# ViktorNfa/bluerov2_dynamics

Measured on AMD Instinct MI355X. Metric: rk4_rollout_steps_per_s, higher is better.
Workload: dtype f64; 1 GPU; BASELINE config 2: 65536 trajectories/GPU x 5000 RK4 steps, thruster model, dt=0.02, iid U(-1,1) commands (splitmix64 stream 0x5EED), layout tpb, all states stored; trajectories_per_gpu=65536, horizon=5000, parallelism=1 x independent shards, no collective

## Files before the change

bluerov2_dynamics_amd/csrc/brov2_fast.h:

```cpp
#pragma once
#include "brov2_device.h"

namespace brov {

struct FastParams {
    double E[12];
    double da[6], db[6];
    double G[5];
    double lc[4][3];
    double ld[4];
    double Tm[6][8];
    double minv[6];
    double poly[5];
    double A1[9], b1[3];
    double A4[9], b4[3];
    double Ob[9];
    double al4[3];
    double Aw4[9], bw4[3];
    double g1[3];
    double XY[4];
    double cur[3];
    int has_current;
    int has_xy;
    int tm_dense;
    int obs_bad;
};

typedef const FastParams __attribute__((address_space(4)))* CFP;
__device__ __forceinline__ CFP as_constant(const FastParams* g) { return (CFP)(unsigned long long)g; }

template <bool RES>
struct HotConstsT {
    static constexpr bool RESIDENT = RES;
    double E[12], db[6];
    double da[6], G[5], ld[4], al4[3];
    double tk[2];
};
typedef HotConstsT<false> HotConsts;
typedef HotConstsT<true> HotConstsResident;

#ifndef BROV_CLAMP_BRANCH
#define BROV_CLAMP_BRANCH 1
#endif
#ifndef BROV_PSI_FRAME
#define BROV_PSI_FRAME 1
#endif
#define BROV_PIN_V(x) asm volatile("" : "+v"(x))
#define BROV_PIN_S(x) asm volatile("" : "+s"(x))
#define BROV_FORM_HERE(r) asm volatile("" : "+v"(r))
#define BROV_SC(h, p, f) (HC::RESIDENT ? (h).f : (p)->f)

template <bool RES>
__device__ __forceinline__ void load_hot(CFP pp, HotConstsT<RES>& h) {
    const auto& p = *pp;
#pragma unroll
    for (int i = 0; i < 12; ++i) { h.E[i] = p.E[i]; BROV_PIN_V(h.E[i]); }
#pragma unroll
    for (int i = 0; i < 6; ++i) { h.db[i] = p.db[i]; BROV_PIN_V(h.db[i]); }
    if constexpr (RES) {
#pragma unroll
        for (int i = 0; i < 6; ++i) { h.da[i] = p.da[i]; BROV_PIN_S(h.da[i]); }
#pragma unroll
        for (int i = 0; i < 5; ++i) { h.G[i] = p.G[i]; BROV_PIN_S(h.G[i]); }
#pragma unroll
        for (int i = 0; i < 4; ++i) { h.ld[i] = p.ld[i]; BROV_PIN_S(h.ld[i]); }
#pragma unroll
        for (int i = 0; i < 3; ++i) { h.al4[i] = p.al4[i]; BROV_PIN_S(h.al4[i]); }
        h.tk[0] = -1.98412698298579493134e-04; BROV_PIN_V(h.tk[0]);
        h.tk[1] = 2.48015872894767294178e-05;  BROV_PIN_V(h.tk[1]);
    }
}

template <bool GENERIC, class HC>
__device__ __forceinline__ const double* trig_consts(const HC& h) {
    if constexpr (HC::RESIDENT && !GENERIC) return h.tk; else return nullptr;
}

__device__ __forceinline__ CFP relaunder(CFP p) {
    asm volatile("" : "+s"(p));
    return p;
}

__device__ __forceinline__ void sincos_fast(double x, double& s, double& c, const double2* __restrict__ qt, const double* kv = nullptr) {
    const double S7 = kv ? kv[0] : -1.98412698298579493134e-04, C8 = kv ? kv[1] : 2.48015872894767294178e-05;
    const double kf = rint(x * 6.36619772367581382433e-01);
    double r = fma(-kf, 1.57079632673412561417e+00, x);
    r = fma(-kf, 6.07710050630396597660e-11, r);
    r = fma(-kf, 2.02226624879595063154e-21, r);
    const int q = (int)kf;
    const double z = r * r;
    double ps = fma(z, 1.58969099521155010221e-10, -2.50507602534068634195e-08);
    ps = fma(z, ps, 2.75573137070700676789e-06);
    ps = fma(z, ps, S7);
    ps = fma(z, ps, 8.33333333332248946124e-03);
    ps = fma(z, ps, -1.66666666666666324348e-01);
    const double sr = fma(z * r, ps, r);
    double pc = fma(z, -1.13596475577881948265e-11, 2.08757232129817482790e-09);
    pc = fma(z, pc, -2.75573143513906633035e-07);
    pc = fma(z, pc, C8);
    pc = fma(z, pc, -1.38888888888741095749e-03);
    pc = fma(z, pc, 4.16666666666666019037e-02);
    const double cr = fma(z * z, pc, fma(-0.5, z, 1.0));
    const double2 t = qt[q & 3];
    s = fma(cr, t.y, sr * t.x);
    c = fma(-sr, t.y, cr * t.x);
}

__device__ __forceinline__ void init_quadrant_table(double2* qt) {
    if (threadIdx.x < 4) {
        const int q = threadIdx.x;
        qt[q] = make_double2(q == 0 ? 1.0 : (q == 2 ? -1.0 : 0.0), q == 1 ? 1.0 : (q == 3 ? -1.0 : 0.0));
    }
}

struct Trig { double sphi, cphi, sth, cth, spsi, cpsi; };

__device__ __forceinline__ void trig_full(const double* ang, Trig& t, const double2* __restrict__ qt, const double* kv = nullptr) {
    sincos_fast(ang[0], t.sphi, t.cphi, qt, kv);
    sincos_fast(ang[1], t.sth, t.cth, qt, kv);
    sincos_fast(ang[2], t.spsi, t.cpsi, qt, kv);
}

template <bool SHORT = false, bool LEAN = false>
__device__ __forceinline__ void trig_delta(const Trig& b, double d[3], Trig& t, double* dpsi = nullptr, const double* kv = nullptr) {
    constexpr int K0 = SHORT ? 4 : 3;
    const double S7 = kv ? kv[0] : -1.98412698298579493134e-04, C8 = kv ? kv[1] : 2.48015872894767294178e-05;
    double dcopy[3] = {d[0], d[1], d[2]};
    double* dd = LEAN ? d : dcopy;
    int k = 0;
    const double m = fmax(fmax(fabs(d[0]), fabs(d[1])), fabs(d[2]));
    const bool far = !(m <= (SHORT ? 0.0625 : 0.125));
    if (far) {
        double mf = m;
        if constexpr (LEAN) asm volatile("; trig_delta range extension, rare" : "+v"(mf));
        int e;
        (void)frexp(mf, &e);
        k = e + K0;
        double sc = ldexp(1.0, -k);
        if (!(mf < 0x1p37)) { sc = __builtin_nan(""); k = 0; }
#pragma unroll
        for (int i = 0; i < 3; ++i) dd[i] *= sc;
    }
    double sd[3], cm[3];
#pragma unroll
    for (int i = 0; i < 3; ++i) {
        const double z = dd[i] * dd[i];
        double ps, pc;
        if constexpr (SHORT) {
            ps = fma(z, S7, 8.33333333332248946124e-03);
            pc = fma(z, C8, -1.38888888888741095749e-03);
        } else {
            ps = fma(z, 2.75573137070700676789e-06, S7);
            ps = fma(z, ps, 8.33333333332248946124e-03);
            pc = fma(z, -2.75573143513906633035e-07, C8);
            pc = fma(z, pc, -1.38888888888741095749e-03);
        }
        ps = fma(z, ps, -1.66666666666666324348e-01);
        sd[i] = fma(z * dd[i], ps, dd[i]);
        pc = fma(z, pc, 4.16666666666666019037e-02);
        pc = fma(z, pc, -0.5);
        cm[i] = z * pc;
    }
    auto doubling = [&](int n) {
        for (int j = 0; j < n; ++j) {
#pragma unroll
            for (int i = 0; i < 3; ++i) {
                const double t2 = sd[i] + sd[i];
                const double s2 = fma(t2, cm[i], t2);
                cm[i] = -(t2 * sd[i]);
                sd[i] = s2;
            }
        }
    };
    if constexpr (LEAN) {
        if (far) {
            double mf = m;
            asm volatile("; trig_delta doubling, rare" : "+v"(mf));
            int e;
            (void)frexp(mf, &e);
            doubling((mf < 0x1p37) ? e + K0 : 0);
        }
    } else doubling(k);
    t.sphi = fma(b.cphi, sd[0], fma(b.sphi, cm[0], b.sphi)); t.cphi = fma(-b.sphi, sd[0], fma(b.cphi, cm[0], b.cphi));
    t.sth = fma(b.cth, sd[1], fma(b.sth, cm[1], b.sth));     t.cth = fma(-b.sth, sd[1], fma(b.cth, cm[1], b.cth));
    t.spsi = fma(b.cpsi, sd[2], fma(b.spsi, cm[2], b.spsi)); t.cpsi = fma(-b.spsi, sd[2], fma(b.cpsi, cm[2], b.cpsi));
    if (dpsi) { dpsi[0] = sd[2]; dpsi[1] = cm[2]; }
}

#ifndef BROV_TRIG_SHORT
#define BROV_TRIG_SHORT 1
#endif
__device__ __forceinline__ double recip_fast(double x) {
    double y = __builtin_amdgcn_rcp(x);
    double e = fma(-x, y, 1.0);
    y = fma(y, e, y);
    e = fma(-x, y, 1.0);
    return fma(y, e, y);
}

template <bool GENERIC, class HC>
__device__ __forceinline__ void nu_dot_fast(const HC& h, CFP p, const double R[9], const double nu[6],
                                            const double a[6], double sth, double ctsp, double ctcp, double out[6]) {
    const double u = nu[0], v = nu[1], w = nu[2], pp = nu[3], q = nu[4], r = nu[5];
    double nr0 = u, nr1 = v, nr2 = w;
    if (GENERIC && p->has_current) {
        nr0 -= fma(R[6], p->cur[2], fma(R[3], p->cur[1], R[0] * p->cur[0]));
        nr1 -= fma(R[7], p->cur[2], fma(R[4], p->cur[1], R[1] * p->cur[0]));
        nr2 -= fma(R[8], p->cur[2], fma(R[5], p->cur[1], R[2] * p->cur[0]));
    }
    double o0 = fma(-h.E[0], w * q, a[0]);  o0 = fma(h.E[1], v * r, o0);
    double o1 = fma(-h.E[2], u * r, a[1]);  o1 = fma(h.E[3], w * pp, o1);
    double o2 = fma(-h.E[4], v * pp, a[2]); o2 = fma(h.E[5], u * q, o2);
    double o3 = fma(-h.E[6], v * w, a[3]);  o3 = fma(-h.E[7], q * r, o3);
    double o4 = fma(-h.E[8], u * w, a[4]);  o4 = fma(-h.E[9], pp * r, o4);
    double o5 = fma(-h.E[10], u * v, a[5]); o5 = fma(-h.E[11], pp * q, o5);
    o0 = fma(-fma(h.db[0], fabs(nr0), BROV_SC(h, p, da[0])), nr0, o0);
    o1 = fma(-fma(h.db[1], fabs(nr1), BROV_SC(h, p, da[1])), nr1, o1);
    o2 = fma(-fma(h.db[2], fabs(nr2), BROV_SC(h, p, da[2])), nr2, o2);
    o3 = fma(-fma(h.db[3], fabs(pp), BROV_SC(h, p, da[3])), pp, o3);
    o4 = fma(-fma(h.db[4], fabs(q), BROV_SC(h, p, da[4])), q, o4);
    o5 = fma(-fma(h.db[5], fabs(r), BROV_SC(h, p, da[5])), r, o5);
    o0 = fma(-BROV_SC(h, p, G[0]), sth, o0);
    o1 = fma(BROV_SC(h, p, G[1]), ctsp, o1);
    o2 = fma(BROV_SC(h, p, G[2]), ctcp, o2);
    o3 = fma(BROV_SC(h, p, G[3]), ctsp, o3);
    o4 = fma(BROV_SC(h, p, G[4]), sth, o4);
    if (GENERIC && p->has_xy) {
        o3 = fma(-p->XY[0], ctcp, o3);
        o4 = fma(p->XY[1], ctcp, o4);
        o5 = fma(-p->XY[2], ctsp, o5);
        o5 = fma(-p->XY[3], sth, o5);
    }
    out[0] = o0; out[1] = o1; out[2] = o2; out[3] = o3; out[4] = o4; out[5] = o5;
}

template <bool GENERIC, class HC, bool PFRAME = false>
__device__ __forceinline__ void rhs_fast_euler(const HC& h, CFP p, const double x[12], const double a[6], double xd[12], const Trig& tg) {
    const double sphi = tg.sphi, cphi = tg.cphi, sth = tg.sth, cth = tg.cth, spsi = tg.spsi, cpsi = tg.cpsi;
    const double* nu = x + 6;
    const double ctsp = cth * sphi, ctcp = cth * cphi;
    if constexpr (GENERIC) {
        double R[9];
        const double ss = sth * sphi, sc = sth * cphi;
        R[0] = cpsi * cth; R[1] = fma(cpsi, ss, -(spsi * cphi)); R[2] = fma(cpsi, sc, spsi * sphi);
        R[3] = spsi * cth; R[4] = fma(spsi, ss, cpsi * cphi);    R[5] = fma(spsi, sc, -(cpsi * sphi));
        R[6] = -sth;       R[7] = ctsp;                          R[8] = ctcp;
        nu_dot_fast<true>(h, p, R, nu, a, sth, ctsp, ctcp, xd + 6);
#pragma unroll
        for (int i = 0; i < 3; ++i) xd[i] = fma(R[3 * i + 2], nu[2], fma(R[3 * i + 1], nu[1], R[3 * i] * nu[0]));
    } else {
        nu_dot_fast<false>(h, p, nullptr, nu, a, sth, ctsp, ctcp, xd + 6);
        const double y1 = fma(cphi, nu[1], -(sphi * nu[2])), z1 = fma(sphi, nu[1], cphi * nu[2]);
        const double x2 = fma(cth, nu[0], sth * z1), z2 = fma(cth, z1, -(sth * nu[0]));
        if constexpr (PFRAME) { xd[0] = x2; xd[1] = y1; }
        else {
            xd[0] = fma(cpsi, x2, -(spsi * y1));
            xd[1] = fma(spsi, x2, cpsi * y1);
        }
        xd[2] = z2;
    }
#if BROV_CLAMP_BRANCH
    double ic = recip_fast(cth);
    if (__builtin_amdgcn_ballot_w64(fabs(cth) < 1e-7) != 0) {
        asm volatile("; cos(theta) clamp, rare" ::: "memory");
        if (fabs(cth) < 1e-7) ic = recip_fast(1e-7 * ((cth > 0.0) - (cth < 0.0)));
    }
#else
    double cc = cth;
    if (fabs(cc) < 1e-7) cc = 1e-7 * ((cc > 0.0) - (cc < 0.0));
    const double ic = recip_fast(cc);
#endif
    const double m = fma(sphi, nu[4], cphi * nu[5]);
    xd[3] = fma(sth * ic, m, nu[3]);
    xd[4] = fma(cphi, nu[4], -(sphi * nu[5]));
    xd[5] = ic * m;
}

template <bool GENERIC, class HC>
__device__ __forceinline__ void rhs_fast_quat(const HC& h, CFP p, const double x[13], const double a[6], double xd[13]) {
    double q[4] = {x[3], x[4], x[5], x[6]};
    quat_normalize(q);
    const double qw = q[0], qx = q[1], qy = q[2], qz = q[3];
    double R[9];
    R[0] = 1.0 - 2.0 * fma(qy, qy, qz * qz); R[1] = 2.0 * fma(qx, qy, -(qz * qw));    R[2] = 2.0 * fma(qx, qz, qy * qw);
    R[3] = 2.0 * fma(qx, qy, qz * qw);       R[4] = 1.0 - 2.0 * fma(qx, qx, qz * qz); R[5] = 2.0 * fma(qy, qz, -(qx * qw));
    R[6] = 2.0 * fma(qx, qz, -(qy * qw));    R[7] = 2.0 * fma(qy, qz, qx * qw);       R[8] = 1.0 - 2.0 * fma(qx, qx, qy * qy);
    const double* nu = x + 7;
    nu_dot_fast<GENERIC>(h, p, R, nu, a, -R[6], R[7], R[8], xd + 7);
#pragma unroll
    for (int i = 0; i < 3; ++i) xd[i] = fma(R[3 * i + 2], nu[2], fma(R[3 * i + 1], nu[1], R[3 * i] * nu[0]));
    const double wx = nu[3], wy = nu[4], wz = nu[5];
    xd[3] = 0.5 * (-(qx * wx) - qy * wy - qz * wz);
    xd[4] = 0.5 * (qw * wx + qy * wz - qz * wy);
    xd[5] = 0.5 * (qw * wy - qx * wz + qz * wx);
    xd[6] = 0.5 * (qw * wz + qx * wy - qy * wx);
}

__device__ __forceinline__ void rhs_di_euler(const double x[12], const double a[6], double xd[12], const Trig& tg) {
    const double sphi = tg.sphi, cphi = tg.cphi, sth = tg.sth, cth = tg.cth, spsi = tg.spsi, cpsi = tg.cpsi;
    const double* v = x + 6;
    const double y1 = fma(cphi, v[1], -(sphi * v[2])), z1 = fma(sphi, v[1], cphi * v[2]);
    const double x2 = fma(cth, v[0], sth * z1);
    xd[0] = fma(cpsi, x2, -(spsi * y1));
    xd[1] = fma(spsi, x2, cpsi * y1);
    xd[2] = fma(cth, z1, -(sth * v[0]));
#pragma unroll
    for (int i = 0; i < 3; ++i) xd[3 + i] = x[9 + i];
#pragma unroll
    for (int i = 0; i < 6; ++i) xd[6 + i] = a[i];
}
__device__ __forceinline__ void rhs_di_quat(const double x[13], const double a[6], double xd[13]) {
    double q[4] = {x[3], x[4], x[5], x[6]};
    quat_normalize(q);
    const double qw = q[0], qx = q[1], qy = q[2], qz = q[3];
    const double R0 = 1.0 - 2.0 * fma(qy, qy, qz * qz), R1 = 2.0 * fma(qx, qy, -(qz * qw)), R2 = 2.0 * fma(qx, qz, qy * qw);
    const double R3 = 2.0 * fma(qx, qy, qz * qw), R4 = 1.0 - 2.0 * fma(qx, qx, qz * qz), R5 = 2.0 * fma(qy, qz, -(qx * qw));
    const double R6 = 2.0 * fma(qx, qz, -(qy * qw)), R7 = 2.0 * fma(qy, qz, qx * qw), R8 = 1.0 - 2.0 * fma(qx, qx, qy * qy);
    const double* v = x + 7;
    xd[0] = fma(R2, v[2], fma(R1, v[1], R0 * v[0]));
    xd[1] = fma(R5, v[2], fma(R4, v[1], R3 * v[0]));
    xd[2] = fma(R8, v[2], fma(R7, v[1], R6 * v[0]));
    const double wx = x[10], wy = x[11], wz = x[12];
    xd[3] = 0.5 * (-(qx * wx) - qy * wy - qz * wz);
    xd[4] = 0.5 * (qw * wx + qy * wz - qz * wy);
    xd[5] = 0.5 * (qw * wy - qx * wz + qz * wx);
    xd[6] = 0.5 * (qw * wz + qx * wy - qy * wx);
#pragma unroll
    for (int i = 0; i < 6; ++i) xd[7 + i] = a[i];
}

template <int MODEL, bool GENERIC, class HC, bool PFRAME = false>
__device__ __forceinline__ void rhs_fast(const HC& h, CFP p, const double* x, const double a[6], double* xd, const Trig& tg) {
    if constexpr (MODEL == MODEL_DI_WRENCH_QUAT) rhs_di_quat(x, a, xd);
    else if constexpr (model_is_di(MODEL)) rhs_di_euler(x, a, xd, tg);
    else if constexpr (MODEL == MODEL_WRENCH_QUAT) rhs_fast_quat<GENERIC>(h, p, x, a, xd);
    else rhs_fast_euler<GENERIC, HC, PFRAME>(h, p, x, a, xd, tg);
}

struct LagZ {
    double z[6][3];
    __device__ __forceinline__ void zero() {
#pragma unroll
        for (int k = 0; k < 6; ++k) { z[k][0] = 0.0; z[k][1] = 0.0; z[k][2] = 0.0; }
    }
    __device__ __forceinline__ void from_thrusters(CFP p, const double X[8][3]) {
#pragma unroll
        for (int k = 0; k < 6; ++k)
#pragma unroll
            for (int j = 0; j < 3; ++j) {
                double a = p->Tm[k][0] * X[0][j];
#pragma unroll
                for (int i = 1; i < 8; ++i) a = fma(p->Tm[k][i], X[i][j], a);
                z[k][j] = a;
            }
    }
    __device__ __forceinline__ void accel_after(CFP p, int s, const double acmd[6], double a[6]) const {
        const double c0 = p->lc[s - 1][0], c1 = p->lc[s - 1][1], c2 = p->lc[s - 1][2], d = p->ld[s - 1];
#pragma unroll
        for (int k = 0; k < 6; ++k) a[k] = fma(c2, z[k][2], fma(c1, z[k][1], fma(c0, z[k][0], d * acmd[k])));
    }
    __device__ __forceinline__ void to_observer(CFP p) {
#pragma unroll
        for (int k = 0; k < 6; ++k) {
            const double a0 = z[k][0], a1 = z[k][1], a2 = z[k][2];
            z[k][0] = fma(p->Ob[2], a2, fma(p->Ob[1], a1, p->Ob[0] * a0));
            z[k][1] = fma(p->Ob[5], a2, fma(p->Ob[4], a1, p->Ob[3] * a0));
            z[k][2] = fma(p->Ob[8], a2, fma(p->Ob[7], a1, p->Ob[6] * a0));
        }
    }
    template <class HC>
    __device__ __forceinline__ void obs_accel_after(const HC& h, CFP p, int s, const double acmd[6], double a[6]) const {
        if (s <= 3) {
            const double d = BROV_SC(h, p, ld[s - 1]);
#pragma unroll
            for (int k = 0; k < 6; ++k) a[k] = fma(d, acmd[k], z[k][s - 1]);
        } else {
            const double c0 = BROV_SC(h, p, al4[0]), c1 = BROV_SC(h, p, al4[1]), c2 = BROV_SC(h, p, al4[2]), d = BROV_SC(h, p, ld[3]);
#pragma unroll
            for (int k = 0; k < 6; ++k) a[k] = fma(c2, z[k][2], fma(c1, z[k][1], fma(c0, z[k][0], d * acmd[k])));
        }
    }
    __device__ __forceinline__ void obs_advance1(CFP p, const double acmd[6]) {
        const double c0 = p->al4[0], c1 = p->al4[1], c2 = p->al4[2], g0 = p->g1[0], g1 = p->g1[1], g2 = p->g1[2];
#pragma unroll
        for (int k = 0; k < 6; ++k) {
            const double a0 = z[k][0], a1 = z[k][1], a2 = z[k][2];
            z[k][0] = fma(g0, acmd[k], a1);
            z[k][1] = fma(g1, acmd[k], a2);
            z[k][2] = fma(c2, a2, fma(c1, a1, fma(c0, a0, g2 * acmd[k])));
        }
    }
    __device__ __forceinline__ void advance(const double __attribute__((address_space(4)))* A, const double __attribute__((address_space(4)))* b, const double acmd[6]) {
#pragma unroll
        for (int k = 0; k < 6; ++k) {
            const double a0 = z[k][0], a1 = z[k][1], a2 = z[k][2];
            const double q0 = fma(A[1], a1, fma(A[0], a0, b[0] * acmd[k]));
            const double q1 = fma(A[4], a1, fma(A[3], a0, b[1] * acmd[k]));
            const double q2 = fma(A[7], a1, fma(A[6], a0, b[2] * acmd[k]));
            double n0 = a0, n1 = a1, n2 = a2;
            asm("v_fma_f64 %0, %1, %2, %3" : "+v"(n0) : "s"(A[2]), "v"(a2), "v"(q0), "v"(q1), "v"(q2));
            asm("v_fma_f64 %0, %1, %2, %3" : "+v"(n1) : "s"(A[5]), "v"(a2), "v"(q1), "v"(q0), "v"(q2));
            asm("v_fma_f64 %0, %1, %0, %2" : "+v"(n2) : "s"(A[8]), "v"(q2), "v"(n0), "v"(n1));
            z[k][0] = n0; z[k][1] = n1; z[k][2] = n2;
        }
    }
};

__device__ __forceinline__ void advance_thrusters(const double __attribute__((address_space(4)))* A, const double __attribute__((address_space(4)))* b, const double fcmd[8], double X[8][3]) {
#pragma unroll
    for (int i = 0; i < 8; ++i) {
        const double a0 = X[i][0], a1 = X[i][1], a2 = X[i][2];
        X[i][0] = fma(A[2], a2, fma(A[1], a1, fma(A[0], a0, b[0] * fcmd[i])));
        X[i][1] = fma(A[5], a2, fma(A[4], a1, fma(A[3], a0, b[1] * fcmd[i])));
        X[i][2] = fma(A[8], a2, fma(A[7], a1, fma(A[6], a0, b[2] * fcmd[i])));
    }
}

template <int MODEL, bool SPARSE>
__device__ __forceinline__ void command_accel(CFP p, const double* u, double fcmd[8], double acmd[6]) {
    if constexpr (MODEL == MODEL_THRUSTER_EULER) {
#pragma unroll
        for (int i = 0; i < 8; ++i) {
            const double V = u[i], V2 = V * V;
            double hh = fma(V2, p->poly[4], p->poly[3]);
            hh = fma(V2, hh, p->poly[2]);
            hh = fma(V2, hh, p->poly[1]);
            hh = fma(V2, hh, p->poly[0]);
            fcmd[i] = V * hh;
        }
        if constexpr (SPARSE) {
#pragma unroll
            for (int k = 0; k < 6; ++k) {
                const int i0 = (k == 2) ? 4 : 0, i1 = (k == 3 || k == 4) ? 8 : (k == 2 ? 8 : 4);
                double a = p->Tm[k][i0] * fcmd[i0];
#pragma unroll
                for (int i = i0 + 1; i < i1; ++i) a = fma(p->Tm[k][i], fcmd[i], a);
                acmd[k] = a;
            }
        } else {
#pragma unroll
            for (int k = 0; k < 6; ++k) {
                double a = p->Tm[k][0] * fcmd[0];
#pragma unroll
                for (int i = 1; i < 8; ++i) a = fma(p->Tm[k][i], fcmd[i], a);
                acmd[k] = a;
            }
        }
    } else if constexpr (model_is_di(MODEL)) {
        constexpr int NU = Dims<MODEL>::NU;
#pragma unroll
        for (int k = 0; k < 6; ++k) {
            double a = p->Tm[k][0] * u[0];
#pragma unroll
            for (int i = 1; i < NU; ++i) a = fma(p->Tm[k][i], u[i], a);
            acmd[k] = a;
        }
    } else {
#pragma unroll
        for (int k = 0; k < 6; ++k) acmd[k] = p->minv[k] * u[k];
    }
}

template <int MODEL, int INTEG, bool GENERIC, class HC, class AccelFn>
__device__ __forceinline__ void integrate_fast(const HC& h, CFP p, double dt, double* x, AccelFn&& accel,
                                               const double2* qt, Trig* carry, bool refresh) {
    constexpr int NX = Dims<MODEL>::NX;
    constexpr bool ANG = !model_is_quat(MODEL);
    constexpr bool LEAN = HC::RESIDENT && !GENERIC;
    double a[6];
    Trig tb, ts;
    const bool CARRY = ANG && carry != nullptr;
    if constexpr (ANG) {
        if (!CARRY || refresh) trig_full(x + 3, tb, qt, trig_consts<GENERIC>(h));
        else tb = *carry;
    }
    double dang[3];
    if constexpr (INTEG == INTEG_EULER) {
        double k[NX];
        accel(1, a);
        rhs_fast<MODEL, GENERIC>(h, p, x, a, k, tb);
        if (CARRY) {
#pragma unroll
            for (int i = 0; i < NX; ++i) {
                if (i >= 3 && i < 6) {
                    if constexpr (LEAN) {
#pragma clang fp contract(off)
                        dang[i - 3] = dt * k[i]; x[i] += dang[i - 3]; BROV_FORM_HERE(x[i]);
                    } else { dang[i - 3] = dt * k[i]; x[i] += dang[i - 3]; }
                } else x[i] = fma(dt, k[i], x[i]);
            }
        } else {
#pragma unroll
            for (int i = 0; i < NX; ++i) x[i] = fma(dt, k[i], x[i]);
        }
    } else {
        double k[NX], xn[NX], xs[NX], dl[3];
        const double h2 = 0.5 * dt, h6 = dt / 6.0, h3 = dt / 3.0;
        constexpr bool PSIF = BROV_PSI_FRAME && ANG && !GENERIC && !model_is_di(MODEL);
        double dps[2] = {0.0, 0.0};
        auto stage_state = [&](double c, auto HALF) {
#pragma unroll
            for (int i = 0; i < NX; ++i) {
                if (ANG && i >= 3 && i < 6) dl[i - 3] = c * k[i];
                else xs[i] = fma(c, k[i], x[i]);
            }
            if constexpr (ANG) trig_delta<BROV_TRIG_SHORT && decltype(HALF)::value, LEAN>(tb, dl, ts, PSIF ? dps : nullptr, trig_consts<GENERIC>(h));
        };
        auto add_turned = [&](double w) {
            const double r0 = fma(dps[1], k[0], fma(-dps[0], k[1], k[0])), r1 = fma(dps[0], k[0], fma(dps[1], k[1], k[1]));
            xn[0] = fma(w, r0, xn[0]);
            xn[1] = fma(w, r1, xn[1]);
        };
        accel(1, a);
        rhs_fast<MODEL, GENERIC, HC, PSIF>(h, p, x, a, k, tb);
#pragma unroll
        for (int i = 0; i < NX; ++i) xn[i] = ((CARRY && i >= 3 && i < 6) || (PSIF && i < 2)) ? h6 * k[i] : fma(h6, k[i], x[i]);
        stage_state(h2, std::true_type{});
        accel(2, a);
        rhs_fast<MODEL, GENERIC, HC, PSIF>(h, p, xs, a, k, ts);
#pragma unroll
        for (int i = PSIF ? 2 : 0; i < NX; ++i) xn[i] = fma(h3, k[i], xn[i]);
        if constexpr (PSIF) add_turned(h3);
        stage_state(h2, std::true_type{});
        accel(3, a);
        rhs_fast<MODEL, GENERIC, HC, PSIF>(h, p, xs, a, k, ts);
#pragma unroll
        for (int i = PSIF ? 2 : 0; i < NX; ++i) xn[i] = fma(h3, k[i], xn[i]);
        if constexpr (PSIF) add_turned(h3);
        stage_state(dt, std::false_type{});
        accel(4, a);
        rhs_fast<MODEL, GENERIC, HC, PSIF>(h, p, xs, a, k, ts);
        if constexpr (PSIF) {
            add_turned(h6);
            x[0] = fma(tb.cpsi, xn[0], fma(-tb.spsi, xn[1], x[0]));
            x[1] = fma(tb.spsi, xn[0], fma(tb.cpsi, xn[1], x[1]));
        }
        if (CARRY) {
#pragma unroll
            for (int i = PSIF ? 2 : 0; i < NX; ++i) {
                if (i >= 3 && i < 6) { dang[i - 3] = fma(h6, k[i], xn[i]); x[i] += dang[i - 3]; if constexpr (LEAN) BROV_FORM_HERE(x[i]); }
                else x[i] = fma(h6, k[i], xn[i]);
            }
        } else {
#pragma unroll
            for (int i = PSIF ? 2 : 0; i < NX; ++i) x[i] = fma(h6, k[i], xn[i]);
        }
    }
    if constexpr (ANG) { if (CARRY) trig_delta<false, LEAN>(tb, dang, *carry, nullptr, trig_consts<GENERIC>(h)); }
    if constexpr (model_is_quat(MODEL)) quat_normalize(x + 3);
}

template <int INTEG, int LAGMODE, bool TRACK, bool GENERIC>
__device__ __forceinline__ void lag_step_advance(CFP pl, LagZ& lz, const double fcmd[8], const double acmd[6], double X[8][3]) {
    constexpr bool OBS = !GENERIC;
    if constexpr (INTEG == INTEG_RK4 && LAGMODE == 0) {
        if constexpr (OBS) lz.advance(pl->Aw4, pl->bw4, acmd); else lz.advance(pl->A4, pl->b4, acmd);
        if constexpr (TRACK) advance_thrusters(pl->A4, pl->b4, fcmd, X);
    } else {
        if constexpr (OBS) lz.obs_advance1(pl, acmd); else lz.advance(pl->A1, pl->b1, acmd);
        if constexpr (TRACK) advance_thrusters(pl->A1, pl->b1, fcmd, X);
    }
}
template <int LAGMODE, bool GENERIC, class HC>
__device__ __forceinline__ void lag_stage_accel(const HC& h, CFP p, const LagZ& lz, int s, const double acmd[6], double a[6]) {
    const int se = LAGMODE == 0 ? s : 1;
    if constexpr (!GENERIC) lz.obs_accel_after(h, p, se, acmd, a); else lz.accel_after(p, se, acmd, a);
}

template <int MODEL, int INTEG, int LAGMODE, bool TRACK, bool GENERIC, class HC>
__device__ __forceinline__ void step_fast(const HC& h, CFP p0, double dt, double* x, const double* u,
                                          LagZ& lz, double X[8][3], const double2* qt, Trig* carry = nullptr, bool refresh = true) {
    constexpr bool THR = (MODEL == MODEL_THRUSTER_EULER);
    CFP p = relaunder(p0);
    double fcmd[8], acmd[6];
    if constexpr (MODEL == MODEL_DI_WRENCH_QUAT) quat_normalize(x + 3);
    command_accel<MODEL, !GENERIC>(p, u, fcmd, acmd);
    integrate_fast<MODEL, INTEG, GENERIC>(h, p, dt, x, [&](int s, double* a) {
        if constexpr (THR) lag_stage_accel<LAGMODE, GENERIC>(h, p, lz, s, acmd, a);
        else {
#pragma unroll
            for (int k = 0; k < 6; ++k) a[k] = acmd[k];
        }
    }, qt, carry, refresh);
    if constexpr (THR) lag_step_advance<INTEG, LAGMODE, TRACK, GENERIC>(relaunder(p0), lz, fcmd, acmd, X);
}

}
```

Before: 28.97 billion steps/s.

## Reorder RK4 stages to compute angle rates first and overlap trig_delta with remaining work

Splits the Euler-angle RHS into the angle-rate part, the body-acceleration part and the position-kinematics part. On the lean resident path each RK4 stage now computes the angle rates first, so the incremental trig update for the next stage can start early. The position and velocity updates are injected as a 'shadow' callback inside trig_delta behind a scheduling barrier, which gives the scheduler independent work to interleave with the sincos polynomial chain. This aims to hide the latency of the serial dependency chain, at the cost of more complex code and possible extra register pressure.

```diff
diff --git a/bluerov2_dynamics_amd/csrc/brov2_fast.h b/bluerov2_dynamics_amd/csrc/brov2_fast.h
--- a/bluerov2_dynamics_amd/csrc/brov2_fast.h
+++ b/bluerov2_dynamics_amd/csrc/brov2_fast.h
@@ -121,8 +121,10 @@
     sincos_fast(ang[2], t.spsi, t.cpsi, qt, kv);
 }
 
-template <bool SHORT = false, bool LEAN = false>
-__device__ __forceinline__ void trig_delta(const Trig& b, double d[3], Trig& t, double* dpsi = nullptr, const double* kv = nullptr) {
+struct NoShadow { __device__ __forceinline__ void operator()() const {} };
+template <bool SHORT = false, bool LEAN = false, class Shadow = NoShadow>
+__device__ __forceinline__ void trig_delta(const Trig& b, double d[3], Trig& t, double* dpsi = nullptr, const double* kv = nullptr,
+                                           Shadow&& shadow = Shadow()) {
     constexpr int K0 = SHORT ? 4 : 3;
     const double S7 = kv ? kv[0] : -1.98412698298579493134e-04, C8 = kv ? kv[1] : 2.48015872894767294178e-05;
     double dcopy[3] = {d[0], d[1], d[2]};
@@ -130,6 +132,10 @@
     int k = 0;
     const double m = fmax(fmax(fabs(d[0]), fabs(d[1])), fabs(d[2]));
     const bool far = !(m <= (SHORT ? 0.0625 : 0.125));
+    if constexpr (!std::is_same<typename std::decay<Shadow>::type, NoShadow>::value) {
+        __builtin_amdgcn_sched_barrier(0);
+        shadow();
+    }
     if (far) {
         double mf = m;
         if constexpr (LEAN) asm volatile("; trig_delta range extension, rare" : "+v"(mf));
@@ -234,8 +240,20 @@
     out[0] = o0; out[1] = o1; out[2] = o2; out[3] = o3; out[4] = o4; out[5] = o5;
 }
 
+template <bool PFRAME>
+__device__ __forceinline__ void euler_pdot(const double nu[6], double xd[12], const Trig& tg) {
+    const double sphi = tg.sphi, cphi = tg.cphi, sth = tg.sth, cth = tg.cth, spsi = tg.spsi, cpsi = tg.cpsi;
+    const double y1 = fma(cphi, nu[1], -(sphi * nu[2])), z1 = fma(sphi, nu[1], cphi * nu[2]);
+    const double x2 = fma(cth, nu[0], sth * z1), z2 = fma(cth, z1, -(sth * nu[0]));
+    if constexpr (PFRAME) { xd[0] = x2; xd[1] = y1; }
+    else {
+        xd[0] = fma(cpsi, x2, -(spsi * y1));
+        xd[1] = fma(spsi, x2, cpsi * y1);
+    }
+    xd[2] = z2;
+}
 template <bool GENERIC, class HC, bool PFRAME = false>
-__device__ __forceinline__ void rhs_fast_euler(const HC& h, CFP p, const double x[12], const double a[6], double xd[12], const Trig& tg) {
+__device__ __forceinline__ void euler_body(const HC& h, CFP p, const double x[12], const double a[6], double xd[12], const Trig& tg) {
     const double sphi = tg.sphi, cphi = tg.cphi, sth = tg.sth, cth = tg.cth, spsi = tg.spsi, cpsi = tg.cpsi;
     const double* nu = x + 6;
     const double ctsp = cth * sphi, ctcp = cth * cphi;
@@ -250,15 +268,11 @@
         for (int i = 0; i < 3; ++i) xd[i] = fma(R[3 * i + 2], nu[2], fma(R[3 * i + 1], nu[1], R[3 * i] * nu[0]));
     } else {
         nu_dot_fast<false>(h, p, nullptr, nu, a, sth, ctsp, ctcp, xd + 6);
-        const double y1 = fma(cphi, nu[1], -(sphi * nu[2])), z1 = fma(sphi, nu[1], cphi * nu[2]);
-        const double x2 = fma(cth, nu[0], sth * z1), z2 = fma(cth, z1, -(sth * nu[0]));
-        if constexpr (PFRAME) { xd[0] = x2; xd[1] = y1; }
-        else {
-            xd[0] = fma(cpsi, x2, -(spsi * y1));
-            xd[1] = fma(spsi, x2, cpsi * y1);
-        }
-        xd[2] = z2;
-    }
+        euler_pdot<PFRAME>(nu, xd, tg);
+    }
+}
+__device__ __forceinline__ void euler_rates(const double nu[6], double xd[12], const Trig& tg) {
+    const double sphi = tg.sphi, cphi = tg.cphi, sth = tg.sth, cth = tg.cth;
 #if BROV_CLAMP_BRANCH
     double ic = recip_fast(cth);
     if (__builtin_amdgcn_ballot_w64(fabs(cth) < 1e-7) != 0) {
@@ -274,6 +288,11 @@
     xd[3] = fma(sth * ic, m, nu[3]);
     xd[4] = fma(cphi, nu[4], -(sphi * nu[5]));
     xd[5] = ic * m;
+}
+template <bool GENERIC, class HC, bool PFRAME = false>
+__device__ __forceinline__ void rhs_fast_euler(const HC& h, CFP p, const double x[12], const double a[6], double xd[12], const Trig& tg) {
+    euler_body<GENERIC, HC, PFRAME>(h, p, x, a, xd, tg);
+    euler_rates(x + 6, xd, tg);
 }
 
 template <bool GENERIC, class HC>
@@ -475,7 +494,126 @@
         else tb = *carry;
     }
     double dang[3];
-    if constexpr (INTEG == INTEG_EULER) {
+    constexpr bool SHADOW = LEAN && ANG && !model_is_di(MODEL);
+    auto pin_accel = [&]() {
+#pragma unroll
+        for (int i = 5; i >= 0; --i) BROV_FORM_HERE(a[i]);
+    };
+    if constexpr (SHADOW && INTEG == INTEG_EULER) {
+        double k[NX];
+        accel(1, a);
+        euler_rates(x + 6, k, tb);
+        pin_accel();
+        nu_dot_fast<false>(h, p, nullptr, x + 6, a, tb.sth, tb.cth * tb.sphi, tb.cth * tb.cphi, k + 6);
+        auto rest = [&]() {
+            euler_pdot<false>(x + 6, k, tb);
+#pragma unroll
+            for (int i = 0; i < NX; ++i) { if (i < 3 || i >= 6) x[i] = fma(dt, k[i], x[i]); }
+#pragma unroll
+            for (int i = 0; i < NX; ++i) { if (i < 3 || i >= 6) BROV_FORM_HERE(x[i]); }
+        };
+        if (CARRY) {
+#pragma unroll
+            for (int i = 3; i < 6; ++i) {
+#pragma clang fp contract(off)
+                dang[i - 3] = dt * k[i]; x[i] += dang[i - 3]; BROV_FORM_HERE(x[i]);
+            }
+            trig_delta<false, LEAN>(tb, dang, *carry, nullptr, trig_consts<GENERIC>(h), rest);
+        } else {
+#pragma unroll
+            for (int i = 3; i < 6; ++i) x[i] = fma(dt, k[i], x[i]);
+            rest();
+        }
+        return;
+    } else if constexpr (SHADOW) {
+        double k[NX], xn[NX], xs[NX], dl[3];
+        const double h2 = 0.5 * dt, h6 = dt / 6.0, h3 = dt / 3.0;
+        constexpr bool PSIF = BROV_PSI_FRAME;
+        double dps[2] = {0.0, 0.0};
+        auto add_turned = [&](double w) {
+            const double r0 = fma(dps[1], k[0], fma(-dps[0], k[1], k[0])), r1 = fma(dps[0], k[0], fma(dps[1], k[1], k[1]));
+            xn[0] = fma(w, r0, xn[0]);
+            xn[1] = fma(w, r1, xn[1]);
+        };
+        auto nu_part = [&](const double* xin, const Trig& tin, int s, double w, double c) {
+            nu_dot_fast<false>(h, p, nullptr, xin + 6, a, tin.sth, tin.cth * tin.sphi, tin.cth * tin.cphi, k + 6);
+#pragma unroll
+            for (int i = 6; i < NX; ++i) xn[i] = (s == 1) ? fma(w, k[i], x[i]) : fma(w, k[i], xn[i]);
+        };
+        auto next_nu = [&](double c) {
+#pragma unroll
+            for (int i = 6; i < NX; ++i) xs[i] = fma(c, k[i], x[i]);
+        };
+        auto pos_part = [&](const double* xin, const Trig& tin, int s, double w) {
+            euler_pdot<PSIF>(xin + 6, k, tin);
+            if (s == 1) {
+#pragma unroll
+                for (int i = 0; i < 3; ++i) xn[i] = (PSIF && i < 2) ? w * k[i] : fma(w, k[i], x[i]);
+            } else {
+#pragma unroll
+                for (int i = PSIF ? 2 : 0; i < 3; ++i) xn[i] = fma(w, k[i], xn[i]);
+                if constexpr (PSIF) add_turned(w);
+            }
+#pragma unroll
+            for (int i = 0; i < 3; ++i) BROV_FORM_HERE(xn[i]);
+        };
+        auto pin_xs = [&]() {
+#pragma unroll
+            for (int i = 6; i < NX; ++i) BROV_FORM_HERE(xs[i]);
+        };
+        auto stage = [&](const double* xin, const Trig& tin, int s, double w, double c, auto HALF) {
+            constexpr bool SH = BROV_TRIG_SHORT && decltype(HALF)::value;
+            if (s == 1) {
+                trig_delta<SH, LEAN>(tb, dl, ts, PSIF ? dps : nullptr, trig_consts<GENERIC>(h), [&]() { pos_part(xin, tin, s, w); });
+                nu_part(xin, tin, s, w, c);
+                next_nu(c);
+            } else {
+                pin_accel();
+                nu_part(xin, tin, s, w, c);
+                trig_delta<SH, LEAN>(tb, dl, ts, PSIF ? dps : nullptr, trig_consts<GENERIC>(h), [&]() { pos_part(xin, tin, s, w); next_nu(c); pin_xs(); });
+            }
+        };
+        accel(1, a);
+        euler_rates(x + 6, k, tb);
+#pragma unroll
+        for (int i = 3; i < 6; ++i) { xn[i] = CARRY ? h6 * k[i] : fma(h6, k[i], x[i]); dl[i - 3] = h2 * k[i]; }
+        stage(x, tb, 1, h6, h2, std::true_type{});
+        accel(2, a);
+        euler_rates(xs + 6, k, ts);
+#pragma unroll
+        for (int i = 3; i < 6; ++i) { xn[i] = fma(h3, k[i], xn[i]); dl[i - 3] = h2 * k[i]; }
+        stage(xs, ts, 2, h3, h2, std::true_type{});
+        accel(3, a);
+        euler_rates(xs + 6, k, ts);
+#pragma unroll
+        for (int i = 3; i < 6; ++i) { xn[i] = fma(h3, k[i], xn[i]); dl[i - 3] = dt * k[i]; }
+        stage(xs, ts, 3, h3, dt, std::false_type{});
+        accel(4, a);
+        euler_rates(xs + 6, k, ts);
+        auto last = [&]() {
+            pin_accel();
+            euler_body<GENERIC, HC, PSIF>(h, p, xs, a, k, ts);
+            if constexpr (PSIF) {
+                add_turned(h6);
+                x[0] = fma(tb.cpsi, xn[0], fma(-tb.spsi, xn[1], x[0]));
+                x[1] = fma(tb.spsi, xn[0], fma(tb.cpsi, xn[1], x[1]));
+            }
+#pragma unroll
+            for (int i = PSIF ? 2 : 0; i < NX; ++i) { if (i < 3 || i >= 6) x[i] = fma(h6, k[i], xn[i]); }
+#pragma unroll
+            for (int i = 6; i < NX; ++i) BROV_FORM_HERE(x[i]);
+        };
+        if (CARRY) {
+#pragma unroll
+            for (int i = 3; i < 6; ++i) { dang[i - 3] = fma(h6, k[i], xn[i]); x[i] += dang[i - 3]; BROV_FORM_HERE(x[i]); }
+            trig_delta<false, LEAN>(tb, dang, *carry, nullptr, trig_consts<GENERIC>(h), last);
+        } else {
+#pragma unroll
+            for (int i = 3; i < 6; ++i) x[i] = fma(h6, k[i], xn[i]);
+            last();
+        }
+        return;
+    } else if constexpr (INTEG == INTEG_EULER) {
         double k[NX];
         accel(1, a);
         rhs_fast<MODEL, GENERIC>(h, p, x, a, k, tb);
```

After: 29.04 billion steps/s, median of 6. No clear change (+0.2%).
